# raulmur/ORB_SLAM

Hardware: NVIDIA H100
Metric: Mkeypoints/s extract+match (higher is better)
Workload: dtype u8

## Files before the change

orb_slam_b200/csrc/extract_kernels.cu:

```cuda
#include <cuda_fp16.h>

#include "orbfe_internal.h"

namespace orbfe {

__global__ void cell_select_harris_kernel(const PlanDev *__restrict__ plan, WorkDev wk, int f0);
__global__ void level_select_harris_kernel(const PlanDev *__restrict__ plan, WorkDev wk, int f0);

__device__ __forceinline__ int find_level_by(const PlanDev *plan, int idx, int which) {
    int l = 0;
    const int n = plan->nlevels;
    for (int k = 1; k < n; k++) {
        const LevelDev &L = plan->lv[k];
        const int base = which == 0 ? L.ftile_base : which == 1 ? L.btile_base : which == 2 ? L.cell_base : L.kp_base;
        if (idx >= base) l = k;
    }
    return l;
}

__device__ __forceinline__ void pdl_prologue() {
    asm volatile("griddepcontrol.launch_dependents;" ::: "memory");
    asm volatile("griddepcontrol.wait;" ::: "memory");
}

// ... 704 lines not shown
        skeys[i] = i < n_out ? (((k & m36) << 8) | (k >> 36)) : 0ull;
    }
    __syncthreads();
    int m2 = 1;
    while (m2 < n_out) m2 <<= 1;
    bitonic_sort_desc(skeys, m2);
    int2 *__restrict__ out = wk.kp_xy_score + (size_t)f * plan->nfeatures + L.kp_base;
    for (int i = threadIdx.x; i < n_out; i += blockDim.x) {
        const unsigned long long k = skeys[i];
        const int score = (int)(k & 0xFF);
        const unsigned long long inv = k >> 8;
        const int cell = 4095 - (int)(inv >> 24);
        const int raster = 0xFFFFFF - (int)(inv & 0xFFFFFF);
        const int ci = cell / L.cols, cj = cell - ci * L.cols;
        const int ly = raster / L.cw, lx = raster - ly * L.cw;
        const int x = ORBFE_EDGE + cj * L.cw + lx, y = ORBFE_EDGE + ci * L.ch + ly;
        out[i] = make_int2(x | (y << 16), score);
    }
    if (threadIdx.x == 0) wk.level_cnt[(size_t)f * plan->nlevels + l] = n_out;
}

__global__ void __launch_bounds__(128) cell_select_harris_kernel(const PlanDev *__restrict__ plan, WorkDev wk, int f0) {
    __shared__ int hist[256];
    __shared__ unsigned long long s_prefix, s_mask;
    __shared__ int s_k, s_base, s_fill;

    const int gcell = blockIdx.x, f = blockIdx.y + f0;
    const size_t fc = (size_t)f * plan->ncells_total + gcell;
    const int keep = wk.cell_keep[fc];
    if (keep <= 0) return;
    const int l = find_level_by(plan, gcell, 2);
    const LevelDev &L = plan->lv[l];
    const int n = min(wk.cell_cnt_lo[fc], wk.cell_cand_cap[gcell]);
    const unsigned long long min_score = wk.cell_min_key[fc] >> 24;
    const unsigned long long *__restrict__ keys = wk.cand_keys64 + (size_t)f * plan->cand_total + wk.cell_cand_base[gcell];
    const int tid = threadIdx.x;
    const int lo = wk.cell_cnt_lo[fc], hi = wk.cell_cnt_hi[fc];
    const int n1 = plan->t1_is_lo ? lo : hi, n2 = plan->t1_is_lo ? hi : lo;
    const int n_elig = (n1 <= 3) ? n2 : n1;

    unsigned long long cut = 0;
    if (n_elig > keep) {
        if (tid == 0) { s_prefix = 0; s_mask = 0; s_k = keep; }
        for (int shift = 56; shift >= 8; shift -= 8) {
            for (int i = tid; i < 256; i += blockDim.x) hist[i] = 0;
            __syncthreads();
            const unsigned long long prefix = s_prefix, mask = s_mask;
            for (int i = tid; i < n; i += blockDim.x) {
                const unsigned long long k = keys[i];
                if ((k & 0xFF) >= min_score && (k & mask) == prefix) atomicAdd(&hist[(int)((k >> shift) & 0xFF)], 1);
            }
            __syncthreads();
            if (tid == 0) {
                int k = s_k, cum = 0, b = 255;
                for (; b >= 0; b--) {
                    if (cum + hist[b] >= k) break;
                    cum += hist[b];
                }
                s_k = k - cum;
                s_prefix = prefix | ((unsigned long long)b << shift);
                s_mask = mask | (0xFFull << shift);
            }
            __syncthreads();
        }
        cut = s_prefix;
    }
    const int nk = min(keep, n_elig);
    if (tid == 0) {
        s_base = atomicAdd(&wk.kept_cnt[(size_t)f * plan->nlevels + l], nk);
        s_fill = 0;
    }
    __syncthreads();
    const int base = s_base;
    const unsigned long long cellinv = (unsigned long long)(4095 - (gcell - L.cell_base));
    unsigned long long *__restrict__ kept = wk.kept_keys + (size_t)f * plan->kept_total + L.kept_base;
    uint32_t *__restrict__ kept2 = wk.kept_aux + (size_t)f * plan->kept_total + L.kept_base;
    for (int i = tid; i < n; i += blockDim.x) {
        const unsigned long long k = keys[i];
        if ((k & 0xFF) >= min_score && (k & ~0xFFull) >= cut) {
            const int p = base + atomicAdd(&s_fill, 1);
            if (p < L.kept_cap) {
                kept[p] = (k & 0xFFFFFFFF00000000ull) | (cellinv << 20) | ((k >> 12) & 0xFFFFFull);
                kept2[p] = (uint32_t)(((k >> 8) & 0xFull) << 8) | (uint32_t)(k & 0xFF);
            } else {
                atomicExch(wk.err_flag, 2);
            }
        }
    }
}

__global__ void __launch_bounds__(512) level_select_harris_kernel(const PlanDev *__restrict__ plan, WorkDev wk, int f0) {
    extern __shared__ unsigned long long skeys[];
    const int l = blockIdx.x, f = blockIdx.y + f0;
    const LevelDev &L = plan->lv[l];
    const int n = min(wk.kept_cnt[(size_t)f * plan->nlevels + l], L.kept_cap);
    uint32_t *slo = reinterpret_cast<uint32_t *>(skeys + L.kept_cap);
    uint8_t *keepf = reinterpret_cast<uint8_t *>(slo + L.kept_cap);
    const unsigned long long *__restrict__ kept = wk.kept_keys + (size_t)f * plan->kept_total + L.kept_base;
    const uint32_t *__restrict__ kept2 = wk.kept_aux + (size_t)f * plan->kept_total + L.kept_base;
    for (int i = threadIdx.x; i < n; i += blockDim.x) { skeys[i] = kept[i]; slo[i] = kept2[i]; }
    __syncthreads();
    const int quota = L.quota;
    for (int i = threadIdx.x; i < n; i += blockDim.x) {
        const unsigned long long hi = skeys[i];
        const uint32_t lo = slo[i] >> 8;
        int rank = 0;
        if (n > quota)
            for (int j = 0; j < n; j++) {
                const unsigned long long hj = skeys[j];
                rank += (hj > hi) || (hj == hi && (slo[j] >> 8) > lo);
            }
        keepf[i] = rank < quota;
    }
    __syncthreads();
    int2 *__restrict__ out = wk.kp_xy_score + (size_t)f * plan->nfeatures + L.kp_base;
    const unsigned long long pos_mask = 0xFFFFFFFFull;
    for (int i = threadIdx.x; i < n; i += blockDim.x) {
        if (!keepf[i]) continue;
        const unsigned long long pi = skeys[i] & pos_mask;
        const uint32_t li = slo[i] >> 8;
        int o = 0;
        for (int j = 0; j < n; j++) {
            if (!keepf[j]) continue;
            const unsigned long long pj = skeys[j] & pos_mask;
            o += (pj > pi) || (pj == pi && (slo[j] >> 8) > li);
        }
        const int cell = 4095 - (int)((pi >> 20) & 0xFFF);
        const int raster = 0xFFFFFF - (int)(((pi & 0xFFFFF) << 4) | li);
        const int ci = cell / L.cols, cj = cell - ci * L.cols;
        const int ly = raster / L.cw, lx = raster - ly * L.cw;
        const int x = ORBFE_EDGE + cj * L.cw + lx, y = ORBFE_EDGE + ci * L.ch + ly;
        out[o] = make_int2(x | (y << 16), (int)__float_as_uint(float_from_order_key((uint32_t)(skeys[i] >> 32))));
    }
    if (threadIdx.x == 0) wk.level_cnt[(size_t)f * plan->nlevels + l] = min(n, quota);
}

int level_select_harris_smem_bytes(int max_kept) { return max_kept * (8 + 4 + 1) + 16; }
int set_level_select_harris_smem(int bytes) {
    return (int)cudaFuncSetAttribute(level_select_harris_kernel, cudaFuncAttributeMaxDynamicSharedMemorySize, bytes);
}

int level_select_smem_bytes(int max_kept) {
    int n2 = 1;
    while (n2 < max_kept) n2 <<= 1;
    return n2 * (int)sizeof(unsigned long long);
}

int set_level_select_smem(int bytes) {
    return (int)cudaFuncSetAttribute(level_select_kernel, cudaFuncAttributeMaxDynamicSharedMemorySize, bytes);
}

void launch_level_select(const PlanDev *d_plan, const PlanDev &hp, WorkDev w, size_t smem_bytes, int f0, int nf, cudaStream_t s) {
    dim3 grid(hp.nlevels, nf);
    if (w.cand_keys64) { level_select_harris_kernel<<<grid, 512, smem_bytes, s>>>(d_plan, w, f0); return; }
    launch_k(level_select_kernel, grid, dim3(512), smem_bytes, s, hp.pdl != 0, d_plan, w, f0);
}

#define B2_W ORBFE_BT_W
#define B2_H ORBFE_BT_H
#define B2_PH (B2_H + 6)
#define B2_PS 128

__device__ __forceinline__ int reflect101(int i, int n) {
    if (n == 1) return 0;
    while (i < 0 || i >= n) i = i < 0 ? -i : 2 * (n - 1) - i;
    return i;
}

__device__ __forceinline__ uint32_t blur_round_u8(int s) {
    int q = (s + 0x7FFF + ((s >> 16) & 1)) >> 16;
    return (uint32_t)min(q, 255);
}

__global__ void __launch_bounds__(256) blur7_kernel(const PlanDev *__restrict__ plan, const BTileInfo *__restrict__ btiles, int f0) {
    __shared__ __align__(16) uint8_t pix[B2_PH * B2_PS];

    const int f = blockIdx.y + f0;
    const BTileInfo bt = btiles[blockIdx.x];
    const LevelDev &L = plan->lv[bt.level];
    const int x0 = bt.tx * B2_W, y0 = bt.ty * B2_H;
    const int w = L.w, h = L.h, pitch = L.pitch;
    const uint8_t *__restrict__ img = L.pyr + (size_t)f * L.plane;

    const bool interior = (x0 >= 4) && (x0 + B2_W + 4 <= w) && (y0 >= 3) && (y0 + B2_H + 3 <= h);
    if (interior) {
        for (int i = threadIdx.x; i < B2_PH * 32; i += blockDim.x) {
            const int r = i >> 5, c = i & 31;
            reinterpret_cast<uint32_t *>(pix)[i] =
                __ldg(reinterpret_cast<const uint32_t *>(img + (size_t)(y0 - 3 + r) * pitch + (x0 - 4)) + c);
        }
    } else {
        for (int i = threadIdx.x; i < B2_PH * B2_PS; i += blockDim.x) {
            const int r = i >> 7, c = i & 127;
            const int gy = reflect101(y0 - 3 + r, h);
            const int gx = reflect101(x0 - 4 + c, w);
            pix[i] = __ldg(img + (size_t)gy * pitch + gx);
        }
    }
    __syncthreads();

    const int g = threadIdx.x & 31, seg = threadIdx.x >> 5;
    const uint32_t *col = reinterpret_cast<const uint32_t *>(pix) + (seg * 8) * 32 + g;
    uint32_t A[7], B[7];
#pragma unroll
    for (int r = 0; r < 6; r++) {
        const uint32_t wv = col[r * 32];
        A[r] = __byte_perm(wv, 0, 0x4240);
        B[r] = __byte_perm(wv, 0, 0x4341);
    }
    uint8_t *__restrict__ dst = L.blur + (size_t)blockIdx.y * L.plane;
    const int gx = x0 - 4 + 4 * g;
#pragma unroll
    for (int i = 0; i < 8; i++) {
        {
            const uint32_t wv = col[(6 + i) * 32];
            A[(6 + i) % 7] = __byte_perm(wv, 0, 0x4240);
            B[(6 + i) % 7] = __byte_perm(wv, 0, 0x4341);
        }
#define WR(k) ((i + (k)) % 7)
        const uint32_t VA = 55u * A[WR(3)] + 49u * (A[WR(2)] + A[WR(4)]) + 34u * (A[WR(1)] + A[WR(5)]) + 18u * (A[WR(0)] + A[WR(6)]);
        const uint32_t VB = 55u * B[WR(3)] + 49u * (B[WR(2)] + B[WR(4)]) + 34u * (B[WR(1)] + B[WR(5)]) + 18u * (B[WR(0)] + B[WR(6)]);
#undef WR
        const uint32_t LA = __shfl_up_sync(0xffffffffu, VA, 1), LB = __shfl_up_sync(0xffffffffu, VB, 1);
        const uint32_t RA = __shfl_down_sync(0xffffffffu, VA, 1), RB = __shfl_down_sync(0xffffffffu, VB, 1);
        const int vm3 = (int)(LB & 0xFFFF), vm2 = (int)(LA >> 16), vm1 = (int)(LB >> 16);
        const int v0 = (int)(VA & 0xFFFF), v1 = (int)(VB & 0xFFFF), v2 = (int)(VA >> 16), v3 = (int)(VB >> 16);
        const int v4 = (int)(RA & 0xFFFF), v5 = (int)(RB & 0xFFFF), v6 = (int)(RA >> 16);
        const int s0 = 55 * v0 + 49 * (vm1 + v1) + 34 * (vm2 + v2) + 18 * (vm3 + v3);
        const int s1 = 55 * v1 + 49 * (v0 + v2) + 34 * (vm1 + v3) + 18 * (vm2 + v4);
        const int s2 = 55 * v2 + 49 * (v1 + v3) + 34 * (v0 + v4) + 18 * (vm1 + v5);
        const int s3 = 55 * v3 + 49 * (v2 + v4) + 34 * (v1 + v5) + 18 * (v0 + v6);
        const uint32_t out = blur_round_u8(s0) | (blur_round_u8(s1) << 8) | (blur_round_u8(s2) << 16) | (blur_round_u8(s3) << 24);
        const int gy = y0 + seg * 8 + i;
        if (g >= 1 && g <= 30 && gy < h && gx < w) *reinterpret_cast<uint32_t *>(dst + (size_t)gy * pitch + gx) = out;
    }
}

void launch_blur(const PlanDev *d_plan, const PlanDev &hp, WorkDev w, int f0, int nf, cudaStream_t s) {
    dim3 grid(hp.nbtiles_total, nf);
    blur7_kernel<<<grid, 256, 0, s>>>(d_plan, w.btile_info, f0);
}

__constant__ int c_umax[16] = {15, 15, 15, 15, 14, 14, 14, 13, 13, 12, 11, 10, 9, 8, 6, 3};

__device__ __forceinline__ float fast_atan2_deg(float y, float x) {
    const float scale = (float)(180.0 / 3.14159265358979323846);
    const float p1 = 0.9997878412794807f * scale, p3 = -0.3258083974640975f * scale;
    const float p5 = 0.1555786518463281f * scale, p7 = -0.04432655554792128f * scale;
    const float eps = (float)2.2204460492503131e-16;
    const float ax = fabsf(x), ay = fabsf(y);
    float a;
    if (ax >= ay) {
        const float c = __fdiv_rn(ay, __fadd_rn(ax, eps));
        const float c2 = __fmul_rn(c, c);
        a = __fmul_rn(__fadd_rn(__fmul_rn(__fadd_rn(__fmul_rn(__fadd_rn(__fmul_rn(p7, c2), p5), c2), p3), c2), p1), c);
    } else {
        const float c = __fdiv_rn(ax, __fadd_rn(ay, eps));
        const float c2 = __fmul_rn(c, c);
        a = __fsub_rn(90.f, __fmul_rn(__fadd_rn(__fmul_rn(__fadd_rn(__fmul_rn(__fadd_rn(__fmul_rn(p7, c2), p5), c2), p3), c2), p1), c));
    }
    if (x < 0) a = __fsub_rn(180.f, a);
    if (y < 0) a = __fsub_rn(360.f, a);
    return a;
}

#define DF_R 21
#define DF_ROWS (2 * DF_R + 1)
#define DF_RW 13
#define DF_VR 37
#define DF_VW 24
#define DF_WARP_WORDS (DF_ROWS * DF_RW + 1 + DF_VR * DF_VW)

template <bool CHECK>
__device__ __forceinline__ int brief_byte_fused(const __half2 *pp, float a, float b, int x, int y, int w, int h,
                                                const uint32_t *vpW, int xoff, const uint8_t *ctr) {
    int val = 0;
#pragma unroll
    for (int k = 0; k < 8; k++) {
        int t[2];
#pragma unroll
        for (int e = 0; e < 2; e++) {
            const float2 pf = __half22float2(pp[(k >> 1) * 128 + ((2 * k + e) & 3)]);
            const float px = pf.x, py = pf.y;
            const float fy = __fadd_rn(__fadd_rn(__fmul_rn(px, b), __fmul_rn(py, a)), 12582912.0f);
            const float fx = __fadd_rn(__fsub_rn(__fmul_rn(px, a), __fmul_rn(py, b)), 12582912.0f);
            const int ry = __float_as_int(fy) - 0x4B400000, rx = __float_as_int(fx) - 0x4B400000;
            const int sx = x + rx, sy = y + ry;
            if (!CHECK || (sx >= 0 && sx < w && sy >= 0 && sy < h)) {
                const int c0 = xoff + rx;
                const uint32_t *vw = vpW + (ry + 18) * DF_VW + (c0 >> 1);
                const bool odd = c0 & 1;
                const uint32_t TX = odd ? 0x31221200u : 0x37312212u, TY = odd ? 0x12223137u : 0x00122231u;
                const int s = (int)__dp2a_lo(vw[0], TX, __dp2a_hi(vw[1], TX, __dp2a_lo(vw[2], TY, __dp2a_hi(vw[3], TY, 0u))));
                t[e] = (int)blur_round_u8(s);
            } else {
                t[e] = ctr[ry * (4 * DF_RW) + rx];
            }
        }
        val |= (t[0] < t[1]) << k;
    }
    return val;
}

template <bool PEERS>
__device__ __forceinline__ void describe_fused_body(const PlanDev *__restrict__ plan, const WorkDev &wk,
                                                    const int8_t *__restrict__ g_pattern,
                                                    OrbfeKeyPoint *__restrict__ out_kps,
                                                    uint8_t *__restrict__ out_desc, int *__restrict__ out_counts, int f0,
                                                    const PeerOut &po) {
    __shared__ __align__(16) __half2 pat[512];
    __shared__ __align__(16) uint32_t patch[8 * DF_WARP_WORDS];
    for (int i = threadIdx.x; i < 512; i += blockDim.x) {
        const char2 p = *reinterpret_cast<const char2 *>(g_pattern + 2 * i);
        const int ln = i >> 4, pr = i & 15;
        pat[((pr >> 2) * 32 + ln) * 4 + (pr & 3)] = __floats2half2_rn((float)p.x, (float)p.y);
    }
    __syncthreads();

    const int f = blockIdx.y + f0;
    const int lane = threadIdx.x & 31;
    const int slot = blockIdx.x * (blockDim.x >> 5) + (threadIdx.x >> 5);
    const int nlev = plan->nlevels;
    const int *__restrict__ lcnt = wk.level_cnt + (size_t)f * nlev;
    if (blockIdx.x == 0 && threadIdx.x == 0) {
        int tot = 0;
        for (int k = 0; k < nlev; k++) tot += lcnt[k];
        if (PEERS) { for (int p = 0; p < po.n; p++) po.counts[p][f] = tot; }
        else out_counts[f] = tot;
    }
    if (slot >= plan->nfeatures) return;
    const int base_k = lane < nlev ? plan->lv[lane].kp_base : 0x7FFFFFFF;
    const int cnt_k = lane < nlev ? lcnt[lane] : 0;
    const int l = 31 - __clz(__ballot_sync(0xffffffffu, slot >= base_k));
    const LevelDev &L = plan->lv[l];
    const int idx = slot - __shfl_sync(0xffffffffu, base_k, l);
    if (idx >= __shfl_sync(0xffffffffu, cnt_k, l)) return;
    const int out_idx = idx + warp_sum(lane < l ? cnt_k : 0);

    const int2 kp = wk.kp_xy_score[(size_t)f * plan->nfeatures + slot];
    const int x = kp.x & 0xFFFF, y = kp.x >> 16;
    const int w = L.w, h = L.h, pitch = L.pitch;
    const uint8_t *__restrict__ img = L.pyr + (size_t)f * L.plane;

    uint32_t *rawW = patch + (threadIdx.x >> 5) * DF_WARP_WORDS;
    uint32_t *vpW = rawW + DF_ROWS * DF_RW + 1;
    uint8_t *rawB = reinterpret_cast<uint8_t *>(rawW);

    const int xa = (x - DF_R) & ~3;
    const bool fast = (x >= DF_R) && (x + DF_R < w) && (y >= DF_R) && (y + DF_R < h) && (xa + 4 * DF_RW <= pitch);
    const int off = fast ? ((x - DF_R) & 3) : 0;
    if (fast) {
        const int sub = lane >= DF_RW ? 1 : 0, c = lane - sub * DF_RW;
        constexpr int NS = (DF_ROWS + 1) / 2;
        uint32_t v[NS];
        const uint32_t *src = reinterpret_cast<const uint32_t *>(img + (size_t)(y - DF_R + sub) * pitch + xa) + c;
        const size_t step = (size_t)pitch >> 1;
        if (lane < 2 * DF_RW) {
#pragma unroll
            for (int q = 0; q < NS; q++)
                if (2 * q + sub < DF_ROWS) v[q] = __ldg(src + q * step);
#pragma unroll
            for (int q = 0; q < NS; q++)
                if (2 * q + sub < DF_ROWS) rawW[(2 * q) * DF_RW + lane] = v[q];
        }
    } else {
        for (int i = lane; i < DF_ROWS * 4 * DF_RW; i += 32) {
            const int r = i / (4 * DF_RW), j = i - r * (4 * DF_RW);
            const int gy = reflect101(y - DF_R + r, h);
            const int gx = reflect101(x - DF_R + j, w);
            rawB[i] = __ldg(img + (size_t)gy * pitch + gx);
        }
    }
    __syncwarp();
    const uint8_t *ctr = rawB + DF_R * (4 * DF_RW) + off + DF_R;

    int m10 = 0, m01 = 0;
    {
        const int u = lane - 15;
        const int au = abs(u);
        if (lane < 31) {
            int colsum = 0;
#pragma unroll
            for (int v = -15; v <= 15; v++) {
                const int val = (au <= c_umax[v < 0 ? -v : v]) ? (int)ctr[v * (4 * DF_RW) + u] : 0;
                colsum += val;
                m01 += v * val;
            }
            m10 = u * colsum;
        }
        m10 = warp_sum(m10);
        m01 = warp_sum(m01);
    }
    const float angle = fast_atan2_deg((float)m01, (float)m10);

    if (lane < 24) {
        const uint32_t T0 = 18u | (34u << 8) | (49u << 16) | (55u << 24), T1 = 49u | (34u << 8) | (18u << 16);
        const int half = lane >= 12 ? 1 : 0, cw = lane - 12 * half;
        const int obase = 20 * half;
        const uint32_t *rw = rawW + obase * DF_RW + cw;
        uint32_t *vw = vpW + obase * DF_VW + 2 * cw;
        uint32_t col[3][4];
#define DF_LOAD_BLOCK(dst, g)                                                                               \
        {                                                                                                   \
            const int rmax = DF_ROWS - 1 - obase;                                                           \
            const uint32_t q0 = rw[min(4 * (g), rmax) * DF_RW], q1 = rw[min(4 * (g) + 1, rmax) * DF_RW];     \
            const uint32_t q2 = rw[min(4 * (g) + 2, rmax) * DF_RW], q3 = rw[min(4 * (g) + 3, rmax) * DF_RW]; \
            const uint32_t t0 = __byte_perm(q0, q1, 0x5140), t1 = __byte_perm(q0, q1, 0x7362);               \
            const uint32_t t2 = __byte_perm(q2, q3, 0x5140), t3 = __byte_perm(q2, q3, 0x7362);               \
            dst[0] = __byte_perm(t0, t2, 0x5410); dst[1] = __byte_perm(t0, t2, 0x7632);                       \
            dst[2] = __byte_perm(t1, t3, 0x5410); dst[3] = __byte_perm(t1, t3, 0x7632);                       \
        }
        DF_LOAD_BLOCK(col[0], 0)
        DF_LOAD_BLOCK(col[1], 1)
#pragma unroll
        for (int g = 0; g < 5; g++) {
            DF_LOAD_BLOCK(col[(g + 2) % 3], g + 2)
#pragma unroll
            for (int sft = 0; sft < 4; sft++) {
                const int o = 4 * g + sft;
                uint32_t hv[4];
#pragma unroll
                for (int j = 0; j < 4; j++) {
                    const uint32_t lo = __funnelshift_r(col[g % 3][j], col[(g + 1) % 3][j], 8 * sft);
                    const uint32_t hi = __funnelshift_r(col[(g + 1) % 3][j], col[(g + 2) % 3][j], 8 * sft);
                    hv[j] = __dp4a(lo, T0, __dp4a(hi, T1, 0u));
                }
                if (obase + o < DF_VR)
                    *reinterpret_cast<uint2 *>(vw + o * DF_VW) = make_uint2(__byte_perm(hv[0], hv[1], 0x5410), __byte_perm(hv[2], hv[3], 0x5410));
            }
        }
#undef DF_LOAD_BLOCK
    }
    __syncwarp();

    const float factorPI = (float)(3.14159265358979323846 / 180.f);
    const float th = __fmul_rn(angle, factorPI);
    double sd, cd;
    sincos((double)th, &sd, &cd);
    const float a = (float)cd, b = (float)sd;
    const bool inner = (x >= 18) && (x + 18 < w) && (y >= 18) && (y + 18 < h);
    const int xoff = off + DF_R - 3;
    const int val = inner ? brief_byte_fused<false>(pat + lane * 4, a, b, x, y, w, h, vpW, xoff, ctr)
                          : brief_byte_fused<true>(pat + lane * 4, a, b, x, y, w, h, vpW, xoff, ctr);
    uint32_t word = (uint32_t)val;
    word |= __shfl_down_sync(0xffffffffu, (uint32_t)val, 1) << 8;
    word |= __shfl_down_sync(0xffffffffu, (uint32_t)val, 2) << 16;
    word |= __shfl_down_sync(0xffffffffu, (uint32_t)val, 3) << 24;
    const size_t o = (size_t)f * plan->nfeatures + out_idx;
    if (PEERS) {
        const uint32_t w1 = __shfl_down_sync(0xffffffffu, word, 4), w2 = __shfl_down_sync(0xffffffffu, word, 8);
        const uint32_t w3 = __shfl_down_sync(0xffffffffu, word, 12);
        const float kx = l ? __fmul_rn((float)x, L.scale) : (float)x, ky = l ? __fmul_rn((float)y, L.scale) : (float)y;
        const float resp = wk.cand_keys64 ? __int_as_float(kp.y) : (float)kp.y;
        const uint32_t field = lane == 0 ? __float_as_uint(kx) : lane == 1 ? __float_as_uint(ky) : lane == 2 ? __float_as_uint(L.patch_size)
                             : lane == 3 ? __float_as_uint(angle) : lane == 4 ? __float_as_uint(resp) : lane == 5 ? (uint32_t)l : 0xFFFFFFFFu;
        for (int p = 0; p < po.n; p++) {
            if ((lane & 15) == 0) reinterpret_cast<uint4 *>(po.desc[p] + o * 32)[lane >> 4] = make_uint4(word, w1, w2, w3);
            if (lane < 7) reinterpret_cast<uint32_t *>(po.kps[p] + o)[lane] = field;
        }
        return;
    }
    if ((lane & 3) == 0) reinterpret_cast<uint32_t *>(out_desc + o * 32)[lane >> 2] = word;
    if (lane == 0) {
        OrbfeKeyPoint r;
        r.x = l ? __fmul_rn((float)x, L.scale) : (float)x;
        r.y = l ? __fmul_rn((float)y, L.scale) : (float)y;
        r.size = L.patch_size;
        r.angle = angle;
        r.response = wk.cand_keys64 ? __int_as_float(kp.y) : (float)kp.y;
        r.octave = l;
        r.class_id = -1;
        out_kps[o] = r;
    }
}

__global__ void __launch_bounds__(256) describe_fused_kernel(const PlanDev *__restrict__ plan, WorkDev wk,
                                                             const int8_t *__restrict__ g_pattern,
                                                             OrbfeKeyPoint *__restrict__ out_kps,
                                                             uint8_t *__restrict__ out_desc, int *__restrict__ out_counts, int f0) {
    pdl_prologue();
    PeerOut none;
    none.n = 0;
    describe_fused_body<false>(plan, wk, g_pattern, out_kps, out_desc, out_counts, f0, none);
}

__global__ void __launch_bounds__(256) describe_fused_exchange_kernel(const PlanDev *__restrict__ plan, WorkDev wk,
                                                                      const int8_t *__restrict__ g_pattern, int f0,
                                                                      const __grid_constant__ PeerOut po) {
    if (po.ack_epoch && (int)threadIdx.x < po.n) {
        const long long t0 = clock64();
        unsigned v;
        do {
            asm volatile("ld.acquire.sys.global.u32 %0, [%1];" : "=r"(v) : "l"(po.ack + threadIdx.x) : "memory");
            if ((int)(v - po.ack_epoch) >= 0) break;
            if (clock64() - t0 > 4000000000ll) { atomicExch(po.err, 2); break; }
            __nanosleep(100);
        } while (true);
    }
    __syncthreads();
    describe_fused_body<true>(plan, wk, g_pattern, nullptr, nullptr, nullptr, f0, po);
    __syncthreads();
    if (threadIdx.x == 0) {
        const unsigned total = gridDim.x * gridDim.y;
        unsigned prev;
        asm volatile("atom.add.release.gpu.global.u32 %0, [%1], 1;" : "=r"(prev) : "l"(po.done) : "memory");
        if (prev == total - 1) {
            asm volatile("fence.acq_rel.sys;" ::: "memory");
            *po.done = 0;
            for (int p = 0; p < po.n; p++)
                asm volatile("st.relaxed.sys.global.u32 [%0], %1;" ::"l"(po.flag[p]), "r"(po.epoch) : "memory");
        }
    }
}

void launch_describe_fused(const PlanDev *d_plan, const PlanDev &hp, WorkDev w, const int8_t *d_pattern,
                           OrbfeKeyPoint *d_kps, uint8_t *d_desc, int *d_counts, int f0, int nf, cudaStream_t s, const PeerOut *peers) {
    dim3 grid((hp.nfeatures + 7) / 8, nf);
    if (grid.x == 0) grid.x = 1;
    if (peers && peers->n > 0) { describe_fused_exchange_kernel<<<grid, 256, 0, s>>>(d_plan, w, d_pattern, f0, *peers); return; }
    launch_k(describe_fused_kernel, grid, dim3(256), 0, s, hp.pdl != 0, d_plan, w, d_pattern, d_kps, d_desc, d_counts, f0);
}

}
```

Before: 46.66.

## Process several keypoints per warp in describe kernel with prefetched coordinates

The fused describe kernel now has each warp handle up to four keypoint slots in a grid-stride loop instead of one, so the grid shrinks by the same factor. The per-block setup (pattern conversion into shared memory, level table loads) is amortized across more keypoints. Keypoint coordinates are software-prefetched two iterations ahead to hide global load latency. The cost is fewer blocks and less parallelism for small feature counts, plus a serial per-warp loop that may lengthen the tail.

```diff
diff --git a/orb_slam_b200/csrc/extract_kernels.cu b/orb_slam_b200/csrc/extract_kernels.cu
--- a/orb_slam_b200/csrc/extract_kernels.cu
+++ b/orb_slam_b200/csrc/extract_kernels.cu
@@ -1030,47 +1030,22 @@
     return val;
 }
 
+__device__ __forceinline__ bool df_slot(int slot, int nfeatures, int base_k, int cnt_k, int &l, int &idx) {
+    if (slot >= nfeatures) return false;
+    l = 31 - __clz(__ballot_sync(0xffffffffu, slot >= base_k));
+    idx = slot - __shfl_sync(0xffffffffu, base_k, l);
+    return idx < __shfl_sync(0xffffffffu, cnt_k, l);
+}
+
 template <bool PEERS>
-__device__ __forceinline__ void describe_fused_body(const PlanDev *__restrict__ plan, const WorkDev &wk,
-                                                    const int8_t *__restrict__ g_pattern,
-                                                    OrbfeKeyPoint *__restrict__ out_kps,
-                                                    uint8_t *__restrict__ out_desc, int *__restrict__ out_counts, int f0,
-                                                    const PeerOut &po) {
-    __shared__ __align__(16) __half2 pat[512];
-    __shared__ __align__(16) uint32_t patch[8 * DF_WARP_WORDS];
-    for (int i = threadIdx.x; i < 512; i += blockDim.x) {
-        const char2 p = *reinterpret_cast<const char2 *>(g_pattern + 2 * i);
-        const int ln = i >> 4, pr = i & 15;
-        pat[((pr >> 2) * 32 + ln) * 4 + (pr & 3)] = __floats2half2_rn((float)p.x, (float)p.y);
-    }
-    __syncthreads();
-
-    const int f = blockIdx.y + f0;
-    const int lane = threadIdx.x & 31;
-    const int slot = blockIdx.x * (blockDim.x >> 5) + (threadIdx.x >> 5);
-    const int nlev = plan->nlevels;
-    const int *__restrict__ lcnt = wk.level_cnt + (size_t)f * nlev;
-    if (blockIdx.x == 0 && threadIdx.x == 0) {
-        int tot = 0;
-        for (int k = 0; k < nlev; k++) tot += lcnt[k];
-        if (PEERS) { for (int p = 0; p < po.n; p++) po.counts[p][f] = tot; }
-        else out_counts[f] = tot;
-    }
-    if (slot >= plan->nfeatures) return;
-    const int base_k = lane < nlev ? plan->lv[lane].kp_base : 0x7FFFFFFF;
-    const int cnt_k = lane < nlev ? lcnt[lane] : 0;
-    const int l = 31 - __clz(__ballot_sync(0xffffffffu, slot >= base_k));
+__device__ __forceinline__ void describe_one(const PlanDev *__restrict__ plan, const WorkDev &wk, const __half2 *pat,
+                                             OrbfeKeyPoint *__restrict__ out_kps, uint8_t *__restrict__ out_desc,
+                                             const PeerOut &po, int f, int l, int out_idx, int2 kp, uint32_t *rawW, int lane) {
     const LevelDev &L = plan->lv[l];
-    const int idx = slot - __shfl_sync(0xffffffffu, base_k, l);
-    if (idx >= __shfl_sync(0xffffffffu, cnt_k, l)) return;
-    const int out_idx = idx + warp_sum(lane < l ? cnt_k : 0);
-
-    const int2 kp = wk.kp_xy_score[(size_t)f * plan->nfeatures + slot];
     const int x = kp.x & 0xFFFF, y = kp.x >> 16;
     const int w = L.w, h = L.h, pitch = L.pitch;
     const uint8_t *__restrict__ img = L.pyr + (size_t)f * L.plane;
 
-    uint32_t *rawW = patch + (threadIdx.x >> 5) * DF_WARP_WORDS;
     uint32_t *vpW = rawW + DF_ROWS * DF_RW + 1;
     uint8_t *rawB = reinterpret_cast<uint8_t *>(rawW);
 
@@ -1202,6 +1177,53 @@
     }
 }
 
+#define DF_SLOTS 4
+
+template <bool PEERS>
+__device__ __forceinline__ void describe_fused_body(const PlanDev *__restrict__ plan, const WorkDev &wk,
+                                                    const int8_t *__restrict__ g_pattern,
+                                                    OrbfeKeyPoint *__restrict__ out_kps,
+                                                    uint8_t *__restrict__ out_desc, int *__restrict__ out_counts, int f0,
+                                                    const PeerOut &po) {
+    __shared__ __align__(16) __half2 pat[512];
+    __shared__ __align__(16) uint32_t patch[8 * DF_WARP_WORDS];
+    for (int i = threadIdx.x; i < 512; i += blockDim.x) {
+        const char2 p = *reinterpret_cast<const char2 *>(g_pattern + 2 * i);
+        const int ln = i >> 4, pr = i & 15;
+        pat[((pr >> 2) * 32 + ln) * 4 + (pr & 3)] = __floats2half2_rn((float)p.x, (float)p.y);
+    }
+    __syncthreads();
+
+    const int f = blockIdx.y + f0;
+    const int lane = threadIdx.x & 31;
+    const int nlev = plan->nlevels, nfeat = plan->nfeatures;
+    const int *__restrict__ lcnt = wk.level_cnt + (size_t)f * nlev;
+    if (blockIdx.x == 0 && threadIdx.x == 0) {
+        int tot = 0;
+        for (int k = 0; k < nlev; k++) tot += lcnt[k];
+        if (PEERS) { for (int p = 0; p < po.n; p++) po.counts[p][f] = tot; }
+        else out_counts[f] = tot;
+    }
+    const int base_k = lane < nlev ? plan->lv[lane].kp_base : 0x7FFFFFFF;
+    const int cnt_k = lane < nlev ? lcnt[lane] : 0;
+    const int2 *__restrict__ kps = wk.kp_xy_score + (size_t)f * nfeat;
+    uint32_t *rawW = patch + (threadIdx.x >> 5) * DF_WARP_WORDS;
+    const int first = blockIdx.x * (blockDim.x >> 5) + (threadIdx.x >> 5), stride = gridDim.x * (blockDim.x >> 5);
+    int2 kp = first < nfeat ? kps[first] : make_int2(0, 0);
+    int2 kp_nxt = (DF_SLOTS > 1 && first + stride < nfeat) ? kps[first + stride] : make_int2(0, 0);
+#pragma unroll 1
+    for (int j = 0; j < DF_SLOTS; j++) {
+        const int slot = first + j * stride;
+        const int2 kp_nn = (j + 2 < DF_SLOTS && slot + 2 * stride < nfeat) ? kps[slot + 2 * stride] : make_int2(0, 0);
+        int l, idx;
+        if (df_slot(slot, nfeat, base_k, cnt_k, l, idx))
+            describe_one<PEERS>(plan, wk, pat, out_kps, out_desc, po, f, l, idx + warp_sum(lane < l ? cnt_k : 0), kp, rawW, lane);
+        __syncwarp();
+        kp = kp_nxt;
+        kp_nxt = kp_nn;
+    }
+}
+
 __global__ void __launch_bounds__(256) describe_fused_kernel(const PlanDev *__restrict__ plan, WorkDev wk,
                                                              const int8_t *__restrict__ g_pattern,
                                                              OrbfeKeyPoint *__restrict__ out_kps,
@@ -1243,7 +1265,7 @@
 
 void launch_describe_fused(const PlanDev *d_plan, const PlanDev &hp, WorkDev w, const int8_t *d_pattern,
                            OrbfeKeyPoint *d_kps, uint8_t *d_desc, int *d_counts, int f0, int nf, cudaStream_t s, const PeerOut *peers) {
-    dim3 grid((hp.nfeatures + 7) / 8, nf);
+    dim3 grid((hp.nfeatures + 8 * DF_SLOTS - 1) / (8 * DF_SLOTS), nf);
     if (grid.x == 0) grid.x = 1;
     if (peers && peers->n > 0) { describe_fused_exchange_kernel<<<grid, 256, 0, s>>>(d_plan, w, d_pattern, f0, *peers); return; }
     launch_k(describe_fused_kernel, grid, dim3(256), 0, s, hp.pdl != 0, d_plan, w, d_pattern, d_kps, d_desc, d_counts, f0);
```

New measurement: 46.90, median of 6. No clear change (+0.5%).
